# mandt-lab/PSLD

Measured on AMD Instinct MI355X. Metric: train images/sec, CIFAR-10 PSLD (6ch 32x32) NCSN++ HSM step, higher is better.
Workload: dtype f32

## Files before the change

### include/psld_hip.h

```cpp
#ifndef PSLD_HIP_H
#define PSLD_HIP_H

#if defined(__HIP__) || defined(__HIPCC__)
#include <hip/hip_runtime_api.h>
#else
typedef struct ihipStream_t* hipStream_t;
#endif

#ifdef __cplusplus
extern "C" {
#endif


#define PSLD_ABI_VERSION 14
#define PSLD_COEFF_STRIDE 12

int psld_version(void);
const char* psld_last_error(void);

#define PSLD_MATH_F32 0
#define PSLD_MATH_BF16X6 1
#define PSLD_MATH_BF16X3 2
int psld_set_math_mode(int mode);
int psld_get_math_mode(void);
// ... 108 lines not shown

int psld_conv3x3_wgrad_split_supported(int cout, int cin, int batch, int h, int w);
int psld_conv3x3_wgrad_split_cout_tile(int cout);
int psld_conv3x3_wgrad_split_f32(const float* dy, int lddy, int cout, const float* x, int cin,
                                 const float* x2, int cin2, int batch, int h, int w, float* slabs,
                                 int cin_total, int col0, int nsplit, hipStream_t stream);
int psld_conv3x3_wgrad_xlimb_f32(const float* dy, int lddy, int cout, const void* x_limb, int cin,
                                 const void* x2_limb, int cin2, int batch, int h, int w, float* slabs,
                                 int cin_total, int col0, int nsplit, hipStream_t stream);
int psld_conv3x3_wgrad_wino_supported(int cout, int cin, int cin2, int batch, int h, int w);
int psld_conv3x3_wgrad_wino_nsplit(int cout, int cin_total, int batch, int h, int w);
long long psld_conv3x3_wgrad_wino_ws_bytes(int cout, int cin_total, int nsplit);
int psld_conv3x3_wgrad_wino_f32(const float* dy, int lddy, int cout, const float* x, int cin, const float* x2, int cin2,
                                int batch, int h, int w, float* slabs, int nsplit, float* dw_oihw, int accumulate,
                                float alpha, hipStream_t stream);
int psld_gemm_tn_split_supported(int m, int n, int k);
int psld_gemm_tn_split_f32(int m, int n, int k, const float* a, int lda, const float* b, int ldb,
                           const float* b2, int ldb2, int n2, float* slabs, int ldc, int nsplit, hipStream_t stream);

int psld_gemm_tail_supported(int k, int m, int n);
long long psld_gemm_frag_bytes_tail(int n, int k);
int psld_pack_gemm_frag_tail(const float* b, void* bfrag, int n, int k, long long stride_n, long long stride_k,
                             hipStream_t stream);
long long psld_pack_frag_tail_items(int n, int n0, int n_total, int k, int chunk0, int chunks_total);
int psld_pack_frag_batch_tail(const long long* table_dev, int entries, long long total_items, hipStream_t stream);
int psld_gemm_split_tail_f32(const float* a, int k, int m, const void* bfrag, int n, float* y, int ldy,
                             const psld_epilogue_t* epi, void* workspace, long long ws_bytes, hipStream_t stream);
int psld_gemm_tn_split_tail_supported(int m, int n, int k);
int psld_gemm_tn_split_tail_f32(int m, int n, int k, const float* a, int lda, const float* b, int ldb, float* slabs,
                                int ldc, int nsplit, hipStream_t stream);
// ... 184 lines not shown
```

### psld_amd/_lib.py

```python
from __future__ import annotations

import ctypes as C
import os

_HERE = os.path.dirname(os.path.abspath(__file__))
LIB_PATH = os.environ.get("PSLD_HIP_LIB") or os.path.join(_HERE, "libpsld_hip.so")

c_f32p = C.c_void_p
c_f64p = C.c_void_p
c_stream = C.c_void_p
c_ll = C.c_longlong


class Epilogue(C.Structure):
    _fields_ = [
        ("alpha", C.c_float),
        ("bias", C.c_void_p),
        ("rowbias", C.c_void_p),
        ("ld_rowbias", C.c_int),
        ("rows_per_img", C.c_int),
        ("residual", C.c_void_p),
        ("ld_residual", C.c_int),
        ("residual_stride_batch", C.c_longlong),
        ("out_scale", C.c_float),
# ... 75 lines not shown
    "psld_pack_gemm_frag": (I, [P, P, I, I, LL, LL, P]),
    "psld_gemm_split_f32": (I, [P, I, P, I, I, P, I, P, I, EP, P, LL, P]),
    "psld_gemm_frag_bytes_x3": (LL, [I, I]),
    "psld_gemm_split_x3_supported": (I, [I, I, I, I]),
    "psld_pack_gemm_frag_x3": (I, [P, P, I, I, LL, LL, P]),
    "psld_pack_frag_batch_x3": (I, [P, I, LL, P]),
    "psld_gemm_split_x3_f32": (I, [P, I, P, I, I, P, I, P, I, EP, P]),
    "psld_conv3x3_wgrad_split_supported": (I, [I, I, I, I, I]),
    "psld_conv3x3_wgrad_split_cout_tile": (I, [I]),
    "psld_conv3x3_wgrad_split_f32": (I, [P, I, I, P, I, P, I, I, I, I, P, I, I, I, P]),
    "psld_conv3x3_wgrad_xlimb_f32": (I, [P, I, I, P, I, P, I, I, I, I, P, I, I, I, P]),
    "psld_conv3x3_wgrad_wino_supported": (I, [I, I, I, I, I, I]),
    "psld_conv3x3_wgrad_wino_nsplit": (I, [I, I, I, I, I]),
    "psld_conv3x3_wgrad_wino_ws_bytes": (LL, [I, I, I]),
    "psld_conv3x3_wgrad_wino_f32": (I, [P, I, I, P, I, P, I, I, I, I, P, I, P, I, F, P]),
    "psld_gemm_tn_split_supported": (I, [I, I, I]),
    "psld_gemm_tn_split_f32": (I, [I, I, I, P, I, P, I, P, I, I, P, I, I, P]),
    "psld_gemm_tail_supported": (I, [I, I, I]),
    "psld_gemm_frag_bytes_tail": (LL, [I, I]),
    "psld_pack_gemm_frag_tail": (I, [P, P, I, I, LL, LL, P]),
    "psld_pack_frag_tail_items": (LL, [I, I, I, I, I, I]),
    "psld_pack_frag_batch_tail": (I, [P, I, LL, P]),
    "psld_gemm_split_tail_f32": (I, [P, I, I, P, I, P, I, EP, P, LL, P]),
    "psld_gemm_tn_split_tail_supported": (I, [I, I, I]),
    "psld_gemm_tn_split_tail_f32": (I, [I, I, I, P, I, P, I, P, I, I, P]),
    "psld_bgemm_split_supported": (I, [I, I, I, I, I]),
    "psld_bgemm_split_f32": (I, [I, I, I, I, I, P, I, LL, P, I, LL, P, I, LL, I, F, P]),
    "psld_reduce_slabs_f32": (I, [P, I, LL, P, I, I, I, I, F, P]),
    "psld_pack_oihw_to_ohwi_f32": (I, [P, P, I, I, I, P]),
    "psld_pack_oihw_to_dgrad_f32": (I, [P, P, I, I, I, P]),
# ... 124 lines not shown
```

### psld_amd/csrc/wgrad_wino.hip

```cpp
#include "limb.h"
#include "psld_hip.h"
#include "tile_shared.h"

namespace {

typedef __attribute__((ext_vector_type(4))) short s16x4;
__device__ __forceinline__ u32x2 lds_tr16(const unsigned char* p) {
    const s16x4 v = __builtin_amdgcn_ds_read_tr16_b64_v4i16(
        (__attribute__((address_space(3))) s16x4*)(__attribute__((address_space(3))) void*)(p));
    return __builtin_bit_cast(u32x2, v);
}

constexpr int WW_CI = 128;
constexpr int WW_RSB = WW_CI * 2 + 32;
constexpr int WW_BLIMB = 32 * WW_RSB;
template <int CO>
struct WWGeom {
    static constexpr int RSA = CO * 2 + 32;
    static constexpr int ALIMB = 32 * RSA;
    static constexpr int IMG = 3 * (ALIMB + WW_BLIMB);
    static constexpr size_t LDS = 2 * (size_t)IMG;
    static constexpr int NY = CO / 32;
    static constexpr int CB = CO / 32;
};
// ... 2 lines not shown
    const float* dy;
    int lddy;
    const float* x;
    int cin;
    const float* x2;
    int cin2;
    int H, W;
    int lg_tw, th_mask, tw_mask;
    int rows_per_kt;
    int lg_kpr, kpr_mask;
    int cout_tiles, cin_tiles;
    int ktiles, ktiles_per_split;
    float* slabs;
    int cout, cin_total;
    int pos_override;
};

__device__ __forceinline__ void x_combo(int i, int& r1, int& r2, float& s) {
    r1 = i == 0 ? 0 : (i == 2 ? 2 : 1);
    r2 = i == 0 ? 2 : (i == 2 ? 1 : (i == 3 ? 3 : 2));
    s = i == 1 ? 1.f : -1.f;
}
__device__ __forceinline__ void y_combo(int i, int& r1, int& n, float& s) {
    r1 = i == 3 ? 1 : 0;
    n = (i == 1 || i == 2) ? 2 : 1;
    s = i == 2 ? -1.f : 1.f;
}

typedef __attribute__((ext_vector_type(2))) float ww_f32x2;
__device__ __forceinline__ unsigned ww_cvt_pk(float a, float b) {
    const ww_f32x2 v = {a, b};
// ... 17 lines not shown
        ww_split3(v[0], v[1], h0, m0, l0);
        ww_split3(v[2], v[3], h1, m1, l1);
    }
    *reinterpret_cast<u32x2*>(d) = u32x2{h0, h1};
    *reinterpret_cast<u32x2*>(d + limb_stride) = u32x2{m0, m1};
    *reinterpret_cast<u32x2*>(d + 2 * limb_stride) = u32x2{l0, l1};
}

__device__ __forceinline__ f32x4 bload(const __amdgpu_buffer_rsrc_t& r, unsigned off) {
    return __builtin_bit_cast(f32x4, __builtin_amdgcn_raw_buffer_load_b128(r, off, 0, 0));
}
__device__ __forceinline__ __amdgpu_buffer_rsrc_t brsrc(const float* p) {
    return __builtin_amdgcn_make_buffer_rsrc(const_cast<float*>(p), 0, 0x7fffffff, 0x00020000);
}

template <int ABL = 0, int CO = 256, bool TAIL = false>
__global__ void __launch_bounds__(512) wwgrad_ws_kernel(const WWgradArgs a) {
    using G = WWGeom<CO>;
    constexpr int WW_CO = CO, WW_RSA = G::RSA, WW_ALIMB = G::ALIMB, WW_IMG = G::IMG, NY = G::NY, CB = G::CB;
    extern __shared__ __attribute__((aligned(16))) unsigned char smem[];
    const int tid = threadIdx.x;
    const int lane = tid & 63, wave = __builtin_amdgcn_readfirstlane(tid >> 6);

    const int units = 16 * a.cin_tiles * a.cout_tiles;
    const int vid = xcd_remap(blockIdx.x, gridDim.x);
    const int split = vid / units;
    int rest = vid - split * units;
    int pos = rest & 15;
    if constexpr (ABL != 0) {
        if (a.pos_override >= 0) pos = a.pos_override;
    }
    rest >>= 4;
    const int ci_tile = rest % a.cin_tiles, co_tile = rest / a.cin_tiles;
    const int pi = pos >> 2, pj = pos & 3;
    const int co0 = co_tile * WW_CO, ci_out = ci_tile * WW_CI;
    const int kt_beg = split * a.ktiles_per_split;
    const int nkt = min(a.ktiles_per_split, a.ktiles - kt_beg);

    if (wave >= 4) {
        const bool second = ci_out >= a.cin;
        const float* xsrc = second ? a.x2 : a.x;
        const int xc = second ? a.cin2 : a.cin;
        const int ci0 = second ? ci_out - a.cin : ci_out;
        const int pt = tid & 255;
        int xr1, xr2, xc1, xc2, yr1, ynr, yc1, ync;
        float xsr, xsc, ysr, ysc;
        x_combo(pi, xr1, xr2, xsr);
        x_combo(pj, xc1, xc2, xsc);
        y_combo(pi, yr1, ynr, ysr);
        y_combo(pj, yc1, ync, ysc);
        const bool need_top = xr1 == 0, need_bot = xr2 == 3;
        const int qx = pt & 31, kx0 = pt >> 5;
        unsigned xoff[4];
        int xdr[4];
        unsigned xcol[4];
#pragma unroll
// ... 20 lines not shown
            }
        }
        const int lds_x = kx0 * WW_RSB + qx * 8, lds_y = ky0 * WW_RSA + qy * 8;

        auto stage = [&](auto nr_tag, auto nc_tag) {
            constexpr int NR = decltype(nr_tag)::value, NC = decltype(nc_tag)::value, NL = NR * NC;
            f32x4 sx[4][4];
            f32x4 sy[NY][NL];
            auto load_tile = [&](int kt) {
                const int kc = kt & a.kpr_mask;
                const int R0 = (kt >> a.lg_kpr) * a.rows_per_kt;
                const int px0 = kc * 64;
                const float* xb = xsrc + ((long long)(2 * R0 - 1) * a.W + px0 - 1) * xc + ci0;
                const __amdgpu_buffer_rsrc_t r11 = brsrc(xb + (long long)(xr1 * a.W + xc1) * xc), r12 = brsrc(xb + (long long)(xr1 * a.W + xc2) * xc),
                                             r21 = brsrc(xb + (long long)(xr2 * a.W + xc1) * xc), r22 = brsrc(xb + (long long)(xr2 * a.W + xc2) * xc);
                const float* yb = a.dy + ((long long)(2 * R0) * a.W + px0) * a.lddy + co0;
                const __amdgpu_buffer_rsrc_t q00 = brsrc(yb + (long long)(yr1 * a.W + yc1) * a.lddy), q01 = brsrc(yb + (long long)(yr1 * a.W + 1) * a.lddy),
                                             q10 = brsrc(yb + (long long)(a.W + yc1) * a.lddy), q11 = brsrc(yb + (long long)(a.W + 1) * a.lddy);
                return [=, &sx, &sy](auto is_x, int i) {
                    if constexpr (decltype(is_x)::value) {
                        const int ty = (R0 + xdr[i]) & a.th_mask;
                        const bool row1 = !(need_top && ty == 0), row2 = !(need_bot && ty == a.th_mask);
                        const bool c1 = (xcol[i] & 1u) != 0 || kc != 0, c2 = (xcol[i] & 2u) != 0 || kc != a.kpr_mask;
                        sx[i][0] = bload(r11, (row1 && c1) ? xoff[i] : 0xffffffffu);
                        sx[i][1] = bload(r12, (row1 && c2) ? xoff[i] : 0xffffffffu);
                        sx[i][2] = bload(r21, (row2 && c1) ? xoff[i] : 0xffffffffu);
                        sx[i][3] = bload(r22, (row2 && c2) ? xoff[i] : 0xffffffffu);
                    } else {
                        sy[i][0] = bload(q00, yoff[i]);
                        if constexpr (NC == 2) sy[i][1] = bload(q01, yoff[i]);
                        if constexpr (NR == 2) {
// ... 139 lines not shown
                    for (int l = 0; l < 3; ++l)
#pragma unroll
                        for (int e = 0; e < 4; ++e) acc[cb][nb][e] += __uint_as_float(fa[cb & 1][l][e] ^ fb[nb][l][e]);
            } else {
#pragma unroll
                for (int u = 0; u < 6; ++u)
#pragma unroll
                    for (int nb = 0; nb < 4; ++nb)
                        acc[cb][nb] = __builtin_amdgcn_mfma_f32_16x16x32_bf16(
                            __builtin_bit_cast(bf16x8, fa[cb & 1][PA[u]]), __builtin_bit_cast(bf16x8, fb[nb][PB[u]]), acc[cb][nb], 0, 0, 0);
            }
        }
        __syncthreads();
    }

    float* S = a.slabs + ((long long)split * 16 + pos) * a.cout * a.cin_total;
#pragma unroll
    for (int cb = 0; cb < CB; ++cb)
#pragma unroll
        for (int nb = 0; nb < 4; ++nb)
#pragma unroll
            for (int v = 0; v < 4; ++v) {
                const int co = co0 + wr * (CO / 2) + cb * 16 + 4 * g + v;
                if (!TAIL || (co < a.cout && ci_out + wc * 64 + nb * 16 + i16 < a.cin_total))
                    S[(long long)co * a.cin_total + ci_out + wc * 64 + nb * 16 + i16] = acc[cb][nb][v];
            }
}

__global__ void __launch_bounds__(64) wwgrad_reduce_kernel(const float* __restrict__ slabs, int nsplit, long long n, float* __restrict__ dw,
                                                           int accumulate, float alpha) {
    const long long idx = (long long)blockIdx.x * 64 + threadIdx.x;
    if (idx >= n) return;
    float m[16];
#pragma unroll
    for (int p = 0; p < 16; ++p) m[p] = 0.f;
    const float* src = slabs + idx;
    for (int sp = 0; sp < nsplit; ++sp) {
        float v[16];
#pragma unroll
        for (int p = 0; p < 16; ++p) v[p] = __builtin_nontemporal_load(src + ((long long)sp * 16 + p) * n);
#pragma unroll
        for (int p = 0; p < 16; ++p) m[p] += v[p];
    }
    float t[4][3];
#pragma unroll
    for (int i = 0; i < 4; ++i) {
        const float h = 0.5f * (m[4 * i + 1] + m[4 * i + 2]), d = 0.5f * (m[4 * i + 1] - m[4 * i + 2]);
        t[i][0] = m[4 * i] + h;
        t[i][1] = d;
        t[i][2] = h - m[4 * i + 3];
    }
    float o[9];
#pragma unroll
    for (int kx = 0; kx < 3; ++kx) {
        const float h = 0.5f * (t[1][kx] + t[2][kx]), d = 0.5f * (t[1][kx] - t[2][kx]);
        o[kx] = t[0][kx] + h;
        o[3 + kx] = d;
        o[6 + kx] = h - t[3][kx];
    }
    float* out = dw + idx * 9;
#pragma unroll
    for (int e = 0; e < 9; ++e) out[e] = accumulate ? out[e] + alpha * o[e] : alpha * o[e];
}

inline int ww_co_tile(int cout) { return cout % 256 ? 128 : 256; }

int ilog2(int v) {
    int l = 0;
    while ((1 << l) < v) ++l;
    return l;
}

}

static bool ww_width_ok(int c) { return c >= 128 && c % 32 == 0; }

extern "C" int psld_conv3x3_wgrad_wino_supported(int cout, int cin, int cin2, int batch, int h, int w) {
// ... 11 lines not shown
    if (n == 0) {
        int dev = 0;
        if (hipGetDevice(&dev) != hipSuccess || hipDeviceGetAttribute(&n, hipDeviceAttributeMultiprocessorCount, dev) != hipSuccess || n <= 0) n = 256;
    }
    int ns = n / units;
    if (ns < 1) ns = 1;
    if (ns > ktiles) ns = (int)ktiles;
    const long long per = (ktiles + ns - 1) / ns;
    return (int)((ktiles + per - 1) / per);
}

extern "C" long long psld_conv3x3_wgrad_wino_ws_bytes(int cout, int cin_total, int nsplit) {
    return (long long)nsplit * 16 * cout * cin_total * 4;
}

extern "C" int psld_conv3x3_wgrad_wino_f32(const float* dy, int lddy, int cout, const float* x, int cin, const float* x2, int cin2,
                                           int batch, int h, int w, float* slabs, int nsplit, float* dw_oihw, int accumulate,
                                           float alpha, hipStream_t stream) {
    PSLD_CHECK_ARG(dy && x && slabs && dw_oihw && nsplit >= 1 && (cin2 == 0 || x2), "psld_conv3x3_wgrad_wino_f32: bad args");
    PSLD_CHECK_ARG(psld_conv3x3_wgrad_wino_supported(cout, cin, cin2, batch, h, w),
                   "psld_conv3x3_wgrad_wino_f32: unsupported shape cout=%d cin=%d+%d B=%d %dx%d", cout, cin, cin2, batch, h, w);
    PSLD_CHECK_ARG(aligned16(dy) && aligned16(x) && (cin2 == 0 || aligned16(x2)) && lddy % 4 == 0 && lddy >= cout,
                   "psld_conv3x3_wgrad_wino_f32: unaligned operand");
    const long long ktiles = (long long)batch * h * w / 4 / 32;
    const long long per_split = (ktiles + nsplit - 1) / nsplit;
    PSLD_CHECK_ARG((ktiles + per_split - 1) / per_split == nsplit, "psld_conv3x3_wgrad_wino_f32: %d splits of %lld K tiles leave empty slabs", nsplit, ktiles);
    WWgradArgs a{};
    a.dy = dy; a.lddy = lddy; a.x = x; a.cin = cin; a.x2 = x2; a.cin2 = cin2;
    a.H = h; a.W = w;
    const int tw = w / 2 < 32 ? w / 2 : 32;
    a.lg_tw = ilog2(tw); a.tw_mask = tw - 1; a.th_mask = h / 2 - 1;
    a.rows_per_kt = 32 >> a.lg_tw;
    a.lg_kpr = ilog2(w / 2 / tw); a.kpr_mask = w / 2 / tw - 1;
    const int co_tile = ww_co_tile(cout);
    a.cout_tiles = (int)cdiv(cout, co_tile); a.cin_tiles = (int)cdiv(cin + cin2, WW_CI);
    const bool tail = cout % co_tile || (cin + cin2) % WW_CI;
    a.ktiles = (int)ktiles; a.ktiles_per_split = (int)per_split;
    a.slabs = slabs; a.cout = cout; a.cin_total = cin + cin2;
    a.pos_override = -1;
    const dim3 grid((unsigned)(16 * a.cout_tiles * a.cin_tiles * nsplit));
#ifdef PSLD_ABLATIONS
    static const int abl = [] { const char* v = getenv("PSLD_WWGRAD_ABL"); return v ? atoi(v) : 0; }();
    static const int pos_ov = [] { const char* v = getenv("PSLD_WWGRAD_POS"); return v ? atoi(v) : -1; }();
    a.pos_override = pos_ov;
#define WW_ABL_CASE(N)                                                                                                              \
    case N:                                                                                                                         \
        (void)hipFuncSetAttribute(reinterpret_cast<const void*>(&wwgrad_ws_kernel<N, 256>), hipFuncAttributeMaxDynamicSharedMemorySize, (int)WWGeom<256>::LDS); \
        hipLaunchKernelGGL((wwgrad_ws_kernel<N, 256>), grid, dim3(512), WWGeom<256>::LDS, stream, a);                                \
        PSLD_CHECK_LAUNCH("wwgrad_ws_kernel (ablation)");                                                                           \
        launched = true;                                                                                                            \
        break;
    bool launched = false;
    switch (co_tile == 256 && !tail ? abl : 0) {
        WW_ABL_CASE(1) WW_ABL_CASE(2) WW_ABL_CASE(3) WW_ABL_CASE(4) WW_ABL_CASE(8) WW_ABL_CASE(12) WW_ABL_CASE(16) WW_ABL_CASE(32) WW_ABL_CASE(64)
        default: break;
    }
#undef WW_ABL_CASE
    if (!launched)
#endif
    {
    static PsldPerDeviceFlag configured_; bool& configured = configured_.here();
    if (!configured) {
        hipError_t e = hipFuncSetAttribute(reinterpret_cast<const void*>(&wwgrad_ws_kernel<0, 256>), hipFuncAttributeMaxDynamicSharedMemorySize, (int)WWGeom<256>::LDS);
        if (e == hipSuccess)
            e = hipFuncSetAttribute(reinterpret_cast<const void*>(&wwgrad_ws_kernel<0, 128>), hipFuncAttributeMaxDynamicSharedMemorySize, (int)WWGeom<128>::LDS);
        if (e == hipSuccess)
            e = hipFuncSetAttribute(reinterpret_cast<const void*>(&wwgrad_ws_kernel<0, 128, true>), hipFuncAttributeMaxDynamicSharedMemorySize, (int)WWGeom<128>::LDS);
        if (e == hipSuccess)
            e = hipFuncSetAttribute(reinterpret_cast<const void*>(&wwgrad_ws_kernel<0, 256, true>), hipFuncAttributeMaxDynamicSharedMemorySize, (int)WWGeom<256>::LDS);
        if (e != hipSuccess) {
            psld_set_error("psld_conv3x3_wgrad_wino_f32: hipFuncSetAttribute failed: %s", hipGetErrorString(e));
            return PSLD_ERR_LAUNCH;
        }
        configured = true;
    }
    if (tail && co_tile == 256)
        hipLaunchKernelGGL((wwgrad_ws_kernel<0, 256, true>), grid, dim3(512), WWGeom<256>::LDS, stream, a);
    else if (tail)
        hipLaunchKernelGGL((wwgrad_ws_kernel<0, 128, true>), grid, dim3(512), WWGeom<128>::LDS, stream, a);
    else if (co_tile == 256)
        hipLaunchKernelGGL((wwgrad_ws_kernel<0, 256>), grid, dim3(512), WWGeom<256>::LDS, stream, a);
    else
        hipLaunchKernelGGL((wwgrad_ws_kernel<0, 128>), grid, dim3(512), WWGeom<128>::LDS, stream, a);
    PSLD_CHECK_LAUNCH("wwgrad_ws_kernel");
    }
    const long long n = (long long)cout * a.cin_total;
    hipLaunchKernelGGL(wwgrad_reduce_kernel, dim3((unsigned)cdiv(n, 64)), dim3(64), 0, stream, slabs, nsplit, n, dw_oihw, accumulate, alpha);
    PSLD_CHECK_LAUNCH("wwgrad_reduce_kernel");
    return PSLD_OK;
}
```

### psld_amd/ops.py

```python
from __future__ import annotations

import ctypes as C
import functools
import os
from typing import Optional, Sequence, Tuple

import numpy as np
import torch

from . import _lib
from ._lib import Epilogue, EmCoeffs, SdeParams, SscsCoeffs, check

Tensor = torch.Tensor
INV_SQRT2 = float(1.0 / np.sqrt(2.0))


def lib():
    return _lib.load()


_stream_cache = []


def _stream() -> int:
# ... 535 lines not shown
def conv3x3_wgrad_wino(dy: Tensor, cout: int, x: Tensor, dw: Tensor, x2: Optional[Tensor] = None, accumulate: bool = False,
                       slabs: Optional[Tensor] = None, nsplit: Optional[int] = None, alpha: float = 1.0):
    b, h, w, cin = x.shape
    cin2 = x2.shape[-1] if x2 is not None else 0
    ns, wsb = conv3x3_wgrad_wino_plan(cout, cin + cin2, b, h, w)
    if nsplit is not None:
        ns, wsb = nsplit, int(lib().psld_conv3x3_wgrad_wino_ws_bytes(cout, cin + cin2, nsplit))
    if slabs is None:
        slabs = workspace(wsb, x.device)
    assert slabs.numel() * slabs.element_size() >= wsb and dw.is_contiguous() and dw.numel() == cout * (cin + cin2) * 9
    check(lib().psld_conv3x3_wgrad_wino_f32(dy.data_ptr(), cout, cout, x.data_ptr(), cin, _p(x2), cin2, b, h, w,
                                            slabs.data_ptr(), ns, dw.data_ptr(), 1 if accumulate else 0, float(alpha), _stream()),
          "psld_conv3x3_wgrad_wino_f32")


def conv2d_wgrad_nhwc(dy: Tensor, cout: int, x: Tensor, kh: int, kw: int, stride: int, pad: int, oh: int, ow: int,
                      slabs: Tensor, cin_total: int, col0: int, nsplit: int):
    b, ih, iw, cin = x.shape
    check(lib().psld_conv2d_wgrad_nhwc_f32(dy.data_ptr(), cout, cout, x.data_ptr(), cin, b, ih, iw, kh, kw, stride,
                                           pad, oh, ow, slabs.data_ptr(), cin_total, col0, nsplit, _stream()),
          "psld_conv2d_wgrad_nhwc_f32")


def reduce_slabs(slabs: Tensor, nsplit: int, n: int, out: Tensor, layout: int = 0, cout: int = 0, taps: int = 0,
                 cin: int = 0, alpha: float = 1.0):
    check(lib().psld_reduce_slabs_f32(slabs.data_ptr(), nsplit, n, out.data_ptr(), layout, cout, taps, cin, alpha,
                                      _stream()), "psld_reduce_slabs_f32")


def pack_ohwi(w_oihw: Tensor, out: Tensor):
# ... 685 lines not shown
```

### psld_amd/score_fn.py

```python
from __future__ import annotations

import math
import os
from typing import List, Optional

import torch
import torch.nn as nn

from . import ops
from .registry import register_module
from .score_exec import _Exec
from .score_modules import (NIN, AttnBlockpp, Downsample, GaussianFourierProjection, ResnetBlockBigGANpp,
                            _Affine, _conv, _groupnorm, _linear, default_init)
from .score_routes import _pick_nsplit
from .score_tape import _SLAB_FLUSH_BYTES, _CatNode, _Node
from .score_weights import (_frag_entry, _packed_entry, _pfrag_entry, _qkv_entry, _temb_entry, _wfrag_x3_entry, pfrag_tail)
from .weight_cache import Entry, WeightCache

Tensor = torch.Tensor
_ALIGN = 64


class _Pending:

# ... 144 lines not shown
                    in_ch = out_ch
                if self.all_resolutions[lvl] in self.attn_resolutions:
                    modules.append(AttnBlockpp(in_ch, init_scale))
                if lvl != 0:
                    modules.append(rb(in_ch=in_ch, up=True))
            assert not hs_c
            modules.append(_groupnorm(in_ch))
            modules.append(_conv(in_ch, sf.out_ch, 3, init_scale))
        self.all_modules = nn.ModuleList(modules)

        self._init_runtime()
        _ow = os.environ.get("PSLD_OVERLAP_WGRAD")
        self.overlap_wgrad = None if _ow is None else _ow == "1"
        self.side_group = 32
        self.defer_param_grads = True
        _ap = os.environ.get("PSLD_AUTOGRAD_PARAMS")
        self.autograd_params = None if _ap is None else _ap == "1"
        self.use_graphs = os.environ.get("PSLD_GRAPHS", "0") == "1"

    def _init_runtime(self):
        self._flat: Optional[Tensor] = None
        self._flat_grad: Optional[Tensor] = None
        self._offsets = None
        self._wcache = WeightCache({"limb": (ops.pack_frag_batch, 2), "limb_tail": (ops.pack_frag_batch_tail, 2),
                                    "wino": (ops.pack_wino_batch, 2),
                                    "limb_x3": (ops.pack_frag_batch_x3, 2), "wino_x3": (ops.pack_wino_batch_x3, 2),
                                    "qkv_bias": (ops.copy_batch, 1), "temb": (ops.copy_batch, 1)})
        self._anchor = None
        self._reducer = None
        self._posfreq = None
# ... 336 lines not shown
```

### psld_amd/score_tape.py

```python
from __future__ import annotations

import os
from typing import Optional

import numpy as np
import torch
import torch.nn as nn

from . import ops
from . import score_routes as R
from .score_modules import _Affine
from .score_routes import _pick_nsplit
from .score_weights import _built_entry

Tensor = torch.Tensor


class _Node:
    __slots__ = ("v", "g", "gp", "used", "want_gsum", "gsum")

    def __init__(self, v, gp=None, want_gsum=False):
        self.v = v
        self.g = None
        self.gp = gp
# ... 54 lines not shown
        self.side_group = net.side_group
        self.want_dx = False
        mode = ops.math_mode()
        self.split = mode in ("bf16x6", "bf16x3")
        self.x3 = mode == "bf16x3" and not record
        self.limb_planes = os.environ.get("PSLD_LIMB_PLANES", "1") != "0"
        self.fused_attn = os.environ.get("PSLD_FUSED_ATTN", "1") != "0"
        self.gn_bwd_colsum = os.environ.get("PSLD_GN_BWD_COLSUM", "1") == "1"
        self.dx_nchw = None
        self.defer = bool(net.defer_param_grads) and record
        self.dense_batched = False
        self.dense_ok = False
        self.dense_pending = []
        self.pjobs, self.pblocks = [], 0
        self.sjobs, self.sitems, self.sbytes = [], 0, 0

    def push(self, fn, module=None):
        if self.tape is not None:
            self.tape.append((fn, module))

    def g(self, p: nn.Parameter) -> Tensor:
        return self.net._grad_view(p)

    def on_side(self, fn, *tensors):
        if self.side is None:
            fn()
            return
        self.side_queue.append((fn, tensors))
        if len(self.side_queue) >= self.side_group:
            self.flush_side()
# ... 3 lines not shown
            return
        queue, self.side_queue = self.side_queue, []
        ev = torch.cuda.Event()
        cur = torch.cuda.current_stream()
        ev.record(cur)
        self.side.wait_event(ev)
        with torch.cuda.stream(self.side), ops.stream_scope():
            for fn, _ in queue:
                fn()
        for _, tensors in queue:
            for t in tensors:
                if t is not None:
                    t.record_stream(self.side)

    def join_side(self):
        if self.side is not None:
            self.flush_side()
            cur = torch.cuda.current_stream()
            cur.wait_stream(self.side)

    @staticmethod
    def use(node: _Node) -> bool:
        first = not node.used
        node.used = True
        return first

    def defer_param(self, src: Tensor, rows: int, ld: int, c: int, dst1: Tensor, dst2: Optional[Tensor] = None,
                    alpha: float = 1.0, src_off: int = 0):
        if not self.defer:
            ops.param_reduce2(src if src_off == 0 else src.view(-1)[src_off:], None, rows, ld, c, dst1, None, alpha)
# ... 49 lines not shown
            dwcat = net._persist("dwcat", (total, kd))
            ops.gemm_tn_split(hi - lo, kd, b, dtp_all[:, lo:hi], total, act, kd, dwcat[lo:hi], kd, 1)
            rows, first = [], 0
            for o, c, d0 in pend:
                n4 = c * kd // 4
                rows += [dwcat.data_ptr() + 4 * o * kd, self.g(d0.weight).data_ptr(), n4, first]
                first += n4
            ops.copy_batch(net._tables.get(rows, dwcat.device), len(pend), first)
        else:
            for o, c, d0 in pend:
                if o % 4 == 0 and ops.gemm_tn_split_supported(c, kd, b):
                    ops.gemm_tn_split(c, kd, b, dtp_all[:, o:o + c], total, act, kd, self.g(d0.weight), kd, 1)
                else:
                    ops.gemm_raw(1, 0, c, kd, b, dtp_all[:, o:o + c], total, 0, act, kd, 0, self.g(d0.weight), kd, 0)

    def flush_deferred(self):
        self.on_side(self.flush_slabs)
        self.flush_params()
        self.flush_dense()

    def finish_backward(self):
        if self.defer:
            self.flush_deferred()
        self.join_side()

    def gn_backward(self, dy: Tensor, x: Tensor, st, gamma: Tensor, beta: Tensor, dgamma: Tensor, dbeta: Tensor, act: bool,
                    dx: Tensor, accumulate_dx: bool = False, add: Optional[Tensor] = None, add_scale: float = 1.0,
                    drop_p: float = 0.0, seed: int = 0, seed_dev=None, groups: Optional[int] = None,
                    colsum_img: Optional[Tensor] = None, ld_img: int = 0, last_writer_of: Optional[_Node] = None):
        b, h, w, c = x.shape
        pa = self.net._param_arena()
# ... 26 lines not shown
            return True
        return False

    def wgrad(self, dy: Tensor, x: Tensor, conv: _Affine, k: int, stride: int, pad: int, alpha: float = 1.0,
              x2: Optional[Tensor] = None, route: Optional[str] = None):
        b, oh, ow, cout = dy.shape
        c1 = x.shape[-1]
        c2 = x2.shape[-1] if x2 is not None else 0
        cin = c1 + c2
        taps = k * k
        n = cout * taps * cin
        assert x2 is None or self.split, "two-source weight gradients exist on the limb kernels only"
        if route is None and (k, stride, pad) == (3, 1, 1):
            route = R.wgrad_route(self.split, cout, c1, c2, b, oh, ow, isinstance(x, ops.LimbPlanes))
        if route == R.WINO:
            ops.conv3x3_wgrad_wino(dy, cout, x, self.g(conv.weight), x2=x2, alpha=alpha)
            return
        if route == R.LIMB:
            nsplit = R.wgrad_limb_nsplit(cout, cin, b, oh, ow, isinstance(x, ops.LimbPlanes))
            slabs = self.slabs_for(4 * n * nsplit, dy.device)
            ops.conv3x3_wgrad_split(dy, cout, x, slabs, cin, 0, nsplit, x2)
            self.reduce_slabs(slabs, nsplit, n, self.g(conv.weight), layout=1, cout=cout, taps=taps, cin=cin, alpha=alpha)
            return
        pw = R.pointwise_wgrad_route(self.split, cout, c1, c2, b * oh * ow) if (k, stride, pad) == (1, 1, 0) else R.TILE
        if pw != R.TILE:
            nsplit = R._tn_split(cout, cin, b * oh * ow)
            slabs = self.slabs_for(4 * n * nsplit, dy.device)
            if pw == R.LIMB_TAIL:
                ops.gemm_tn_split_tail(cout, c1, b * oh * ow, dy, cout, x, c1, slabs, cin, nsplit)
            else:
                ops.gemm_tn_split(cout, c1, b * oh * ow, dy, cout, x, c1, slabs, cin, nsplit, x2, c2, c2)
# ... 184 lines not shown
```

Measured before the change: 1253.

## Batch same-shape Winograd weight-gradient jobs into one grouped launch

Adds a batched Winograd wgrad kernel that reads per-job dy/x/dw pointers and alpha from a device table. Same-shape wgrad calls are deferred and launched together once a group fills, with fewer K splits per job so each block does more work. The aim is to cut launch count and the tiny-split inefficiency on small spatial layers. In exchange it adds a table-write kernel, larger slab workspace, deferred-tensor lifetime handling and cross-stream record_stream bookkeeping.

After: 1259 (median of 6 runs). No clear change (+0.5%).

```diff
diff --git a/include/psld_hip.h b/include/psld_hip.h
--- a/include/psld_hip.h
+++ b/include/psld_hip.h
@@ -146,6 +146,10 @@
 int psld_conv3x3_wgrad_wino_f32(const float* dy, int lddy, int cout, const float* x, int cin, const float* x2, int cin2,
                                 int batch, int h, int w, float* slabs, int nsplit, float* dw_oihw, int accumulate,
                                 float alpha, hipStream_t stream);
+int psld_conv3x3_wgrad_wino_group(int cout, int cin_total, int batch, int h, int w, int* nsplit);
+int psld_conv3x3_wgrad_wino_batch_f32(const long long* table_dev, int jobs, int lddy, int cout, int cin, int cin2, int batch,
+                                      int h, int w, float* slabs, int nsplit, int accumulate, hipStream_t stream);
+int psld_table_write_i64(long long* table_dev, const long long* rows_host, int count, hipStream_t stream);
 int psld_gemm_tn_split_supported(int m, int n, int k);
 int psld_gemm_tn_split_f32(int m, int n, int k, const float* a, int lda, const float* b, int ldb,
                            const float* b2, int ldb2, int n2, float* slabs, int ldc, int nsplit, hipStream_t stream);
diff --git a/psld_amd/_lib.py b/psld_amd/_lib.py
--- a/psld_amd/_lib.py
+++ b/psld_amd/_lib.py
@@ -113,6 +113,9 @@
     "psld_conv3x3_wgrad_wino_nsplit": (I, [I, I, I, I, I]),
     "psld_conv3x3_wgrad_wino_ws_bytes": (LL, [I, I, I]),
     "psld_conv3x3_wgrad_wino_f32": (I, [P, I, I, P, I, P, I, I, I, I, P, I, P, I, F, P]),
+    "psld_conv3x3_wgrad_wino_group": (I, [I, I, I, I, I, C.POINTER(I)]),
+    "psld_conv3x3_wgrad_wino_batch_f32": (I, [P, I, I, I, I, I, I, I, I, P, I, I, P]),
+    "psld_table_write_i64": (I, [P, P, I, P]),
     "psld_gemm_tn_split_supported": (I, [I, I, I]),
     "psld_gemm_tn_split_f32": (I, [I, I, I, P, I, P, I, P, I, I, P, I, I, P]),
     "psld_gemm_tail_supported": (I, [I, I, I]),
diff --git a/psld_amd/csrc/wgrad_wino.hip b/psld_amd/csrc/wgrad_wino.hip
--- a/psld_amd/csrc/wgrad_wino.hip
+++ b/psld_amd/csrc/wgrad_wino.hip
@@ -40,7 +40,11 @@
     float* slabs;
     int cout, cin_total;
     int pos_override;
+    const long long* table;
+    int nsplit;
 };
+constexpr int WW_ROW = 8;
+typedef const __attribute__((address_space(4))) long long* ww_row_ptr;
 
 __device__ __forceinline__ void x_combo(int i, int& r1, int& r2, float& s) {
     r1 = i == 0 ? 0 : (i == 2 ? 2 : 1);
@@ -88,7 +92,7 @@
     return __builtin_amdgcn_make_buffer_rsrc(const_cast<float*>(p), 0, 0x7fffffff, 0x00020000);
 }
 
-template <int ABL = 0, int CO = 256, bool TAIL = false>
+template <int ABL = 0, int CO = 256, bool TAIL = false, bool BATCH = false>
 __global__ void __launch_bounds__(512) wwgrad_ws_kernel(const WWgradArgs a) {
     using G = WWGeom<CO>;
     constexpr int WW_CO = CO, WW_RSA = G::RSA, WW_ALIMB = G::ALIMB, WW_IMG = G::IMG, NY = G::NY, CB = G::CB;
@@ -98,8 +102,14 @@
 
     const int units = 16 * a.cin_tiles * a.cout_tiles;
     const int vid = xcd_remap(blockIdx.x, gridDim.x);
-    const int split = vid / units;
+    int split = vid / units;
     int rest = vid - split * units;
+    const int slab = split;
+    int job = 0;
+    if constexpr (BATCH) {
+        job = split / a.nsplit;
+        split -= job * a.nsplit;
+    }
     int pos = rest & 15;
     if constexpr (ABL != 0) {
         if (a.pos_override >= 0) pos = a.pos_override;
@@ -113,7 +123,9 @@
 
     if (wave >= 4) {
         const bool second = ci_out >= a.cin;
-        const float* xsrc = second ? a.x2 : a.x;
+        const ww_row_ptr row = (ww_row_ptr)(unsigned long long)a.table + job * WW_ROW;
+        const float* xsrc = BATCH ? reinterpret_cast<const float*>(row[second ? 2 : 1]) : (second ? a.x2 : a.x);
+        const float* dyp = BATCH ? reinterpret_cast<const float*>(row[0]) : a.dy;
         const int xc = second ? a.cin2 : a.cin;
         const int ci0 = second ? ci_out - a.cin : ci_out;
         const int pt = tid & 255;
@@ -164,7 +176,7 @@
                 const float* xb = xsrc + ((long long)(2 * R0 - 1) * a.W + px0 - 1) * xc + ci0;
                 const __amdgpu_buffer_rsrc_t r11 = brsrc(xb + (long long)(xr1 * a.W + xc1) * xc), r12 = brsrc(xb + (long long)(xr1 * a.W + xc2) * xc),
                                              r21 = brsrc(xb + (long long)(xr2 * a.W + xc1) * xc), r22 = brsrc(xb + (long long)(xr2 * a.W + xc2) * xc);
-                const float* yb = a.dy + ((long long)(2 * R0) * a.W + px0) * a.lddy + co0;
+                const float* yb = dyp + ((long long)(2 * R0) * a.W + px0) * a.lddy + co0;
                 const __amdgpu_buffer_rsrc_t q00 = brsrc(yb + (long long)(yr1 * a.W + yc1) * a.lddy), q01 = brsrc(yb + (long long)(yr1 * a.W + 1) * a.lddy),
                                              q10 = brsrc(yb + (long long)(a.W + yc1) * a.lddy), q11 = brsrc(yb + (long long)(a.W + 1) * a.lddy);
                 return [=, &sx, &sy](auto is_x, int i) {
@@ -334,7 +346,7 @@
         __syncthreads();
     }
 
-    float* S = a.slabs + ((long long)split * 16 + pos) * a.cout * a.cin_total;
+    float* S = a.slabs + ((long long)slab * 16 + pos) * a.cout * a.cin_total;
 #pragma unroll
     for (int cb = 0; cb < CB; ++cb)
 #pragma unroll
@@ -348,9 +360,15 @@
 }
 
 __global__ void __launch_bounds__(64) wwgrad_reduce_kernel(const float* __restrict__ slabs, int nsplit, long long n, float* __restrict__ dw,
-                                                           int accumulate, float alpha) {
+                                                           int accumulate, float alpha, const long long* table) {
     const long long idx = (long long)blockIdx.x * 64 + threadIdx.x;
     if (idx >= n) return;
+    if (table) {
+        const ww_row_ptr row = (ww_row_ptr)(unsigned long long)table + blockIdx.y * WW_ROW;
+        dw = reinterpret_cast<float*>(row[3]);
+        alpha = __builtin_bit_cast(float, (unsigned)row[4]);
+        slabs += (long long)blockIdx.y * nsplit * 16 * n;
+    }
     float m[16];
 #pragma unroll
     for (int p = 0; p < 16; ++p) m[p] = 0.f;
@@ -381,6 +399,13 @@
     float* out = dw + idx * 9;
 #pragma unroll
     for (int e = 0; e < 9; ++e) out[e] = accumulate ? out[e] + alpha * o[e] : alpha * o[e];
+}
+
+struct WWRows { long long v[8 * WW_ROW]; };
+__global__ void __launch_bounds__(64) ww_table_write_kernel(long long* __restrict__ table, const WWRows r, int count) {
+#pragma unroll
+    for (int i = 0; i < 8 * WW_ROW; ++i)
+        if ((int)threadIdx.x == i && i < count) table[i] = r.v[i];
 }
 
 inline int ww_co_tile(int cout) { return cout % 256 ? 128 : 256; }
@@ -422,19 +447,34 @@
     return (long long)nsplit * 16 * cout * cin_total * 4;
 }
 
-extern "C" int psld_conv3x3_wgrad_wino_f32(const float* dy, int lddy, int cout, const float* x, int cin, const float* x2, int cin2,
-                                           int batch, int h, int w, float* slabs, int nsplit, float* dw_oihw, int accumulate,
-                                           float alpha, hipStream_t stream) {
-    PSLD_CHECK_ARG(dy && x && slabs && dw_oihw && nsplit >= 1 && (cin2 == 0 || x2), "psld_conv3x3_wgrad_wino_f32: bad args");
+constexpr int WW_GROUP_T = 64;
+
+extern "C" int psld_conv3x3_wgrad_wino_group(int cout, int cin_total, int batch, int h, int w, int* nsplit) {
+    const int ns1 = psld_conv3x3_wgrad_wino_nsplit(cout, cin_total, batch, h, w);
+    if (nsplit) *nsplit = ns1;
+    if (ns1 <= 0) return 0;
+    const long long ktiles = (long long)batch * h * w / 4 / 32;
+    const long long per1 = ktiles / ns1;
+    if (per1 >= WW_GROUP_T || per1 < 1) return 1;
+    int g = (int)((WW_GROUP_T + per1 - 1) / per1);
+    if (g > ns1) g = ns1;
+    if (g > 8) g = 8;
+    int ns = ns1 / g;
+    const long long per = (ktiles + ns - 1) / ns;
+    if (nsplit) *nsplit = (int)((ktiles + per - 1) / per);
+    return g;
+}
+
+namespace {
+
+int ww_fill_args(WWgradArgs& a, const char* who, bool ptrs_aligned, int lddy, int cout, int cin, int cin2, int batch, int h, int w, int nsplit) {
     PSLD_CHECK_ARG(psld_conv3x3_wgrad_wino_supported(cout, cin, cin2, batch, h, w),
-                   "psld_conv3x3_wgrad_wino_f32: unsupported shape cout=%d cin=%d+%d B=%d %dx%d", cout, cin, cin2, batch, h, w);
-    PSLD_CHECK_ARG(aligned16(dy) && aligned16(x) && (cin2 == 0 || aligned16(x2)) && lddy % 4 == 0 && lddy >= cout,
-                   "psld_conv3x3_wgrad_wino_f32: unaligned operand");
+                   "%s: unsupported shape cout=%d cin=%d+%d B=%d %dx%d", who, cout, cin, cin2, batch, h, w);
+    PSLD_CHECK_ARG(ptrs_aligned && lddy % 4 == 0 && lddy >= cout, "%s: unaligned operand", who);
     const long long ktiles = (long long)batch * h * w / 4 / 32;
     const long long per_split = (ktiles + nsplit - 1) / nsplit;
-    PSLD_CHECK_ARG((ktiles + per_split - 1) / per_split == nsplit, "psld_conv3x3_wgrad_wino_f32: %d splits of %lld K tiles leave empty slabs", nsplit, ktiles);
-    WWgradArgs a{};
-    a.dy = dy; a.lddy = lddy; a.x = x; a.cin = cin; a.x2 = x2; a.cin2 = cin2;
+    PSLD_CHECK_ARG((ktiles + per_split - 1) / per_split == nsplit, "%s: %d splits of %lld K tiles leave empty slabs", who, nsplit, ktiles);
+    a.lddy = lddy; a.cin = cin; a.cin2 = cin2;
     a.H = h; a.W = w;
     const int tw = w / 2 < 32 ? w / 2 : 32;
     a.lg_tw = ilog2(tw); a.tw_mask = tw - 1; a.th_mask = h / 2 - 1;
@@ -442,15 +482,60 @@
     a.lg_kpr = ilog2(w / 2 / tw); a.kpr_mask = w / 2 / tw - 1;
     const int co_tile = ww_co_tile(cout);
     a.cout_tiles = (int)cdiv(cout, co_tile); a.cin_tiles = (int)cdiv(cin + cin2, WW_CI);
-    const bool tail = cout % co_tile || (cin + cin2) % WW_CI;
     a.ktiles = (int)ktiles; a.ktiles_per_split = (int)per_split;
-    a.slabs = slabs; a.cout = cout; a.cin_total = cin + cin2;
+    a.cout = cout; a.cin_total = cin + cin2;
     a.pos_override = -1;
-    const dim3 grid((unsigned)(16 * a.cout_tiles * a.cin_tiles * nsplit));
+    a.nsplit = nsplit;
+    return PSLD_OK;
+}
+
+template <bool BATCH>
+int ww_launch(const WWgradArgs& a, const char* who, unsigned blocks, hipStream_t stream) {
+    static PsldPerDeviceFlag configured_; bool& configured = configured_.here();
+    if (!configured) {
+        hipError_t e = hipFuncSetAttribute(reinterpret_cast<const void*>(&wwgrad_ws_kernel<0, 256, false, BATCH>), hipFuncAttributeMaxDynamicSharedMemorySize, (int)WWGeom<256>::LDS);
+        if (e == hipSuccess)
+            e = hipFuncSetAttribute(reinterpret_cast<const void*>(&wwgrad_ws_kernel<0, 128, false, BATCH>), hipFuncAttributeMaxDynamicSharedMemorySize, (int)WWGeom<128>::LDS);
+        if (e == hipSuccess)
+            e = hipFuncSetAttribute(reinterpret_cast<const void*>(&wwgrad_ws_kernel<0, 128, true, BATCH>), hipFuncAttributeMaxDynamicSharedMemorySize, (int)WWGeom<128>::LDS);
+        if (e == hipSuccess)
+            e = hipFuncSetAttribute(reinterpret_cast<const void*>(&wwgrad_ws_kernel<0, 256, true, BATCH>), hipFuncAttributeMaxDynamicSharedMemorySize, (int)WWGeom<256>::LDS);
+        if (e != hipSuccess) {
+            psld_set_error("%s: hipFuncSetAttribute failed: %s", who, hipGetErrorString(e));
+            return PSLD_ERR_LAUNCH;
+        }
+        configured = true;
+    }
+    const dim3 grid(blocks);
+    const int co_tile = ww_co_tile(a.cout);
+    const bool tail = a.cout % co_tile || a.cin_total % WW_CI;
+    if (tail && co_tile == 256)
+        hipLaunchKernelGGL((wwgrad_ws_kernel<0, 256, true, BATCH>), grid, dim3(512), WWGeom<256>::LDS, stream, a);
+    else if (tail)
+        hipLaunchKernelGGL((wwgrad_ws_kernel<0, 128, true, BATCH>), grid, dim3(512), WWGeom<128>::LDS, stream, a);
+    else if (co_tile == 256)
+        hipLaunchKernelGGL((wwgrad_ws_kernel<0, 256, false, BATCH>), grid, dim3(512), WWGeom<256>::LDS, stream, a);
+    else
+        hipLaunchKernelGGL((wwgrad_ws_kernel<0, 128, false, BATCH>), grid, dim3(512), WWGeom<128>::LDS, stream, a);
+    PSLD_CHECK_LAUNCH("wwgrad_ws_kernel");
+    return PSLD_OK;
+}
+
+}
+
+extern "C" int psld_conv3x3_wgrad_wino_f32(const float* dy, int lddy, int cout, const float* x, int cin, const float* x2, int cin2,
+                                           int batch, int h, int w, float* slabs, int nsplit, float* dw_oihw, int accumulate,
+                                           float alpha, hipStream_t stream) {
+    PSLD_CHECK_ARG(dy && x && slabs && dw_oihw && nsplit >= 1 && (cin2 == 0 || x2), "psld_conv3x3_wgrad_wino_f32: bad args");
+    WWgradArgs a{};
+    if (const int st = ww_fill_args(a, "psld_conv3x3_wgrad_wino_f32", aligned16(dy) && aligned16(x) && (cin2 == 0 || aligned16(x2)), lddy, cout, cin, cin2, batch, h, w, nsplit)) return st;
+    a.dy = dy; a.x = x; a.x2 = x2; a.slabs = slabs;
+    const unsigned blocks = (unsigned)(16 * a.cout_tiles * a.cin_tiles * nsplit);
 #ifdef PSLD_ABLATIONS
     static const int abl = [] { const char* v = getenv("PSLD_WWGRAD_ABL"); return v ? atoi(v) : 0; }();
     static const int pos_ov = [] { const char* v = getenv("PSLD_WWGRAD_POS"); return v ? atoi(v) : -1; }();
     a.pos_override = pos_ov;
+    const dim3 grid(blocks);
 #define WW_ABL_CASE(N)                                                                                                              \
     case N:                                                                                                                         \
         (void)hipFuncSetAttribute(reinterpret_cast<const void*>(&wwgrad_ws_kernel<N, 256>), hipFuncAttributeMaxDynamicSharedMemorySize, (int)WWGeom<256>::LDS); \
@@ -459,7 +544,7 @@
         launched = true;                                                                                                            \
         break;
     bool launched = false;
-    switch (co_tile == 256 && !tail ? abl : 0) {
+    switch (ww_co_tile(cout) == 256 && cout % 256 == 0 && (cin + cin2) % WW_CI == 0 ? abl : 0) {
         WW_ABL_CASE(1) WW_ABL_CASE(2) WW_ABL_CASE(3) WW_ABL_CASE(4) WW_ABL_CASE(8) WW_ABL_CASE(12) WW_ABL_CASE(16) WW_ABL_CASE(32) WW_ABL_CASE(64)
         default: break;
     }
@@ -467,33 +552,35 @@
     if (!launched)
 #endif
     {
-    static PsldPerDeviceFlag configured_; bool& configured = configured_.here();
-    if (!configured) {
-        hipError_t e = hipFuncSetAttribute(reinterpret_cast<const void*>(&wwgrad_ws_kernel<0, 256>), hipFuncAttributeMaxDynamicSharedMemorySize, (int)WWGeom<256>::LDS);
-        if (e == hipSuccess)
-            e = hipFuncSetAttribute(reinterpret_cast<const void*>(&wwgrad_ws_kernel<0, 128>), hipFuncAttributeMaxDynamicSharedMemorySize, (int)WWGeom<128>::LDS);
-        if (e == hipSuccess)
-            e = hipFuncSetAttribute(reinterpret_cast<const void*>(&wwgrad_ws_kernel<0, 128, true>), hipFuncAttributeMaxDynamicSharedMemorySize, (int)WWGeom<128>::LDS);
-        if (e == hipSuccess)
-            e = hipFuncSetAttribute(reinterpret_cast<const void*>(&wwgrad_ws_kernel<0, 256, true>), hipFuncAttributeMaxDynamicSharedMemorySize, (int)WWGeom<256>::LDS);
-        if (e != hipSuccess) {
-            psld_set_error("psld_conv3x3_wgrad_wino_f32: hipFuncSetAttribute failed: %s", hipGetErrorString(e));
-            return PSLD_ERR_LAUNCH;
-        }
-        configured = true;
-    }
-    if (tail && co_tile == 256)
-        hipLaunchKernelGGL((wwgrad_ws_kernel<0, 256, true>), grid, dim3(512), WWGeom<256>::LDS, stream, a);
-    else if (tail)
-        hipLaunchKernelGGL((wwgrad_ws_kernel<0, 128, true>), grid, dim3(512), WWGeom<128>::LDS, stream, a);
-    else if (co_tile == 256)
-        hipLaunchKernelGGL((wwgrad_ws_kernel<0, 256>), grid, dim3(512), WWGeom<256>::LDS, stream, a);
-    else
-        hipLaunchKernelGGL((wwgrad_ws_kernel<0, 128>), grid, dim3(512), WWGeom<128>::LDS, stream, a);
-    PSLD_CHECK_LAUNCH("wwgrad_ws_kernel");
+        if (const int st = ww_launch<false>(a, "psld_conv3x3_wgrad_wino_f32", blocks, stream)) return st;
     }
     const long long n = (long long)cout * a.cin_total;
-    hipLaunchKernelGGL(wwgrad_reduce_kernel, dim3((unsigned)cdiv(n, 64)), dim3(64), 0, stream, slabs, nsplit, n, dw_oihw, accumulate, alpha);
+    hipLaunchKernelGGL(wwgrad_reduce_kernel, dim3((unsigned)cdiv(n, 64)), dim3(64), 0, stream, slabs, nsplit, n, dw_oihw, accumulate, alpha,
+                       (const long long*)nullptr);
     PSLD_CHECK_LAUNCH("wwgrad_reduce_kernel");
     return PSLD_OK;
 }
+
+extern "C" int psld_conv3x3_wgrad_wino_batch_f32(const long long* table_dev, int jobs, int lddy, int cout, int cin, int cin2, int batch,
+                                                 int h, int w, float* slabs, int nsplit, int accumulate, hipStream_t stream) {
+    PSLD_CHECK_ARG(table_dev && slabs && jobs >= 1 && jobs <= 8 && nsplit >= 1, "psld_conv3x3_wgrad_wino_batch_f32: bad args");
+    WWgradArgs a{};
+    if (const int st = ww_fill_args(a, "psld_conv3x3_wgrad_wino_batch_f32", true, lddy, cout, cin, cin2, batch, h, w, nsplit)) return st;
+    a.table = table_dev; a.slabs = slabs;
+    if (const int st = ww_launch<true>(a, "psld_conv3x3_wgrad_wino_batch_f32", (unsigned)(16 * a.cout_tiles * a.cin_tiles * nsplit * jobs), stream))
+        return st;
+    const long long n = (long long)cout * a.cin_total;
+    hipLaunchKernelGGL(wwgrad_reduce_kernel, dim3((unsigned)cdiv(n, 64), (unsigned)jobs), dim3(64), 0, stream, slabs, nsplit, n,
+                       (float*)nullptr, accumulate, 0.f, table_dev);
+    PSLD_CHECK_LAUNCH("wwgrad_reduce_kernel");
+    return PSLD_OK;
+}
+
+extern "C" int psld_table_write_i64(long long* table_dev, const long long* rows_host, int count, hipStream_t stream) {
+    PSLD_CHECK_ARG(table_dev && rows_host && count >= 1 && count <= 8 * WW_ROW, "psld_table_write_i64: bad args (count=%d)", count);
+    WWRows r{};
+    for (int i = 0; i < count; ++i) r.v[i] = rows_host[i];
+    hipLaunchKernelGGL(ww_table_write_kernel, dim3(1), dim3(64), 0, stream, table_dev, r, count);
+    PSLD_CHECK_LAUNCH("ww_table_write_kernel");
+    return PSLD_OK;
+}
diff --git a/psld_amd/ops.py b/psld_amd/ops.py
--- a/psld_amd/ops.py
+++ b/psld_amd/ops.py
@@ -573,6 +573,35 @@
           "psld_conv3x3_wgrad_wino_f32")
 
 
+@functools.lru_cache(maxsize=None)
+def conv3x3_wgrad_wino_group_plan(cout: int, cin_total: int, b: int, h: int, w: int):
+    ns = C.c_int(0)
+    g = int(lib().psld_conv3x3_wgrad_wino_group(cout, cin_total, b, h, w, C.byref(ns)))
+    return g, ns.value, int(lib().psld_conv3x3_wgrad_wino_ws_bytes(cout, cin_total, ns.value))
+
+
+def conv3x3_wgrad_wino_batch(jobs, cout: int, nsplit: int, accumulate: bool = False):
+    dy0, x0, x20 = jobs[0][0], jobs[0][1], jobs[0][2]
+    b, h, w, cin = x0.shape
+    cin2 = x20.shape[-1] if x20 is not None else 0
+    n = cout * (cin + cin2) * 9
+    rows = []
+    for dy, x, x2, dw, alpha in jobs:
+        assert dy.shape == dy0.shape and x.shape == x0.shape and (x2 is None) == (x20 is None) and (x2 is None or x2.shape == x20.shape)
+        assert dw.is_contiguous() and dw.numel() == n
+        ptrs = [dy.data_ptr(), x.data_ptr(), _p(x2) or 0, dw.data_ptr()]
+        assert all(p % 16 == 0 for p in ptrs[:3]), "psld_conv3x3_wgrad_wino_batch_f32: unaligned operand"
+        rows += ptrs + [int(np.float32(alpha).view(np.uint32)), 0, 0, 0]
+    wsb = int(lib().psld_conv3x3_wgrad_wino_ws_bytes(cout, cin + cin2, nsplit))
+    slabs = workspace(len(jobs) * wsb, x0.device)
+    table = torch.empty((len(rows),), dtype=torch.int64, device=x0.device)
+    host = (C.c_longlong * len(rows))(*rows)
+    check(lib().psld_table_write_i64(table.data_ptr(), host, len(rows), _stream()), "psld_table_write_i64")
+    check(lib().psld_conv3x3_wgrad_wino_batch_f32(table.data_ptr(), len(jobs), cout, cout, cin, cin2, b, h, w,
+                                                  slabs.data_ptr(), nsplit, 1 if accumulate else 0, _stream()),
+          "psld_conv3x3_wgrad_wino_batch_f32")
+
+
 def conv2d_wgrad_nhwc(dy: Tensor, cout: int, x: Tensor, kh: int, kw: int, stride: int, pad: int, oh: int, ow: int,
                       slabs: Tensor, cin_total: int, col0: int, nsplit: int):
     b, ih, iw, cin = x.shape
diff --git a/psld_amd/score_fn.py b/psld_amd/score_fn.py
--- a/psld_amd/score_fn.py
+++ b/psld_amd/score_fn.py
@@ -182,6 +182,7 @@
         self.overlap_wgrad = None if _ow is None else _ow == "1"
         self.side_group = 32
         self.defer_param_grads = True
+        self.wgrad_group = None
         _ap = os.environ.get("PSLD_AUTOGRAD_PARAMS")
         self.autograd_params = None if _ap is None else _ap == "1"
         self.use_graphs = os.environ.get("PSLD_GRAPHS", "0") == "1"
diff --git a/psld_amd/score_tape.py b/psld_amd/score_tape.py
--- a/psld_amd/score_tape.py
+++ b/psld_amd/score_tape.py
@@ -92,6 +92,8 @@
         self.dense_pending = []
         self.pjobs, self.pblocks = [], 0
         self.sjobs, self.sitems, self.sbytes = [], 0, 0
+        self.wgrad_group = net.wgrad_group
+        self.wpending = {}
 
     def push(self, fn, module=None):
         if self.tape is not None:
@@ -125,6 +127,8 @@
                     t.record_stream(self.side)
 
     def join_side(self):
+        if self.wpending:
+            self.on_side(self.flush_wgroups)
         if self.side is not None:
             self.flush_side()
             cur = torch.cuda.current_stream()
@@ -204,7 +208,29 @@
                 else:
                     ops.gemm_raw(1, 0, c, kd, b, dtp_all[:, o:o + c], total, 0, act, kd, 0, self.g(d0.weight), kd, 0)
 
+    def launch_wgroup(self, key):
+        jobs = self.wpending.pop(key)
+        cout, c1, c2, b, h, w = key
+        _, ns, _ = ops.conv3x3_wgrad_wino_group_plan(cout, c1 + c2, b, h, w)
+        if len(jobs) == 1:
+            dy, x, x2, dw, alpha = jobs[0]
+            ops.conv3x3_wgrad_wino(dy, cout, x, dw, x2=x2, nsplit=ns, alpha=alpha)
+        else:
+            ops.conv3x3_wgrad_wino_batch(jobs, cout, ns)
+        if self.side is not None:
+            cur = torch.cuda.current_stream()
+            for dy, x, x2, _, _ in jobs:
+                for t in (dy, x, x2):
+                    if t is not None:
+                        t.record_stream(cur)
+
+    def flush_wgroups(self):
+        for key in list(self.wpending):
+            self.launch_wgroup(key)
+
     def flush_deferred(self):
+        if self.wpending:
+            self.on_side(self.flush_wgroups)
         self.on_side(self.flush_slabs)
         self.flush_params()
         self.flush_dense()
@@ -261,7 +287,17 @@
         if route is None and (k, stride, pad) == (3, 1, 1):
             route = R.wgrad_route(self.split, cout, c1, c2, b, oh, ow, isinstance(x, ops.LimbPlanes))
         if route == R.WINO:
-            ops.conv3x3_wgrad_wino(dy, cout, x, self.g(conv.weight), x2=x2, alpha=alpha)
+            group, ns, _ = ops.conv3x3_wgrad_wino_group_plan(cout, cin, b, oh, ow)
+            if self.wgrad_group is not None:
+                group = min(group, max(int(self.wgrad_group), 1))
+            if group <= 1 or not self.defer:
+                ops.conv3x3_wgrad_wino(dy, cout, x, self.g(conv.weight), x2=x2, nsplit=ns, alpha=alpha)
+                return
+            key = (cout, c1, c2, b, oh, ow)
+            pend = self.wpending.setdefault(key, [])
+            pend.append((dy, x, x2, self.g(conv.weight), alpha))
+            if len(pend) >= group:
+                self.launch_wgroup(key)
             return
         if route == R.LIMB:
             nsplit = R.wgrad_limb_nsplit(cout, cin, b, oh, ow, isinstance(x, ops.LimbPlanes))
```
